# igashov/DiffLinker

Hardware: AMD Instinct MI355X
Metric: molecules/sec (500-step sample_chain) (higher is better)
Workload: dtype f32 (f16x3 split MFMA, fp32 accumulate)

## Files before the change

### difflinker_amd/csrc/egnn_fc.hip

```cpp
#include <hip/hip_runtime.h>
#include <stdint.h>
#include <stdlib.h>
#include <string.h>
#include <math.h>
#include <cmath>

#include <algorithm>
#include <atomic>
#include <vector>

#include "../../include/difflinker_hip.h"
#include "pack_layout.h"


namespace {

constexpr int LDH = 132;
constexpr int NMAX = 55;
constexpr int NQMAX = 2 * NMAX;
constexpr int THREADS = 512;
constexpr int NWAVES = THREADS / 64;
constexpr int GWAVES = 8;
constexpr int GTHREADS = 64 * GWAVES;
constexpr int L_A = 0;
// ... 1242 lines not shown
        for (int t = 0; t < 4; ++t) { acc[t][0] += __uint_as_float(al[t].x ^ ah[t].y); acc[t][1] += __uint_as_float(al[t].z ^ ah[t].w); }
#else
#pragma unroll
        for (int t = 0; t < 4; ++t) acc[t] = mfma16(al[t], b.hi[sl], acc[t]);
#pragma unroll
        for (int t = 0; t < 4; ++t) acc[t] = mfma16(ah[t], b.lo[sl], acc[t]);
#pragma unroll
        for (int t = 0; t < 4; ++t) acc[t] = mfma16(ah[t], b.hi[sl], acc[t]);
#endif
    }
}
template <int SLOT>
__device__ __forceinline__ void st_issue(float* lds0, const float* __restrict__ src, int hw, int lane) {
    typedef const __attribute__((address_space(1))) void* gptr_t;
    typedef __attribute__((address_space(3))) void* lptr_t;
    const float4* s4 = reinterpret_cast<const float4*>(src) + lane;
#ifdef DL_KO_DMA
    (void)s4; (void)lds0; (void)hw;
#else
#pragma unroll
    for (int it = 0; it < ST_PIECES; ++it) {
        const int piece = it * 4 + hw;
        __builtin_amdgcn_global_load_lds((gptr_t)(s4 + piece * 64), (lptr_t)(lds0 + st_slot_off(SLOT) + piece * 256), 16, 0, 0);
    }
#endif
}
template <int HALF>
__device__ __forceinline__ void st_issue_image(const Lds& v, const NextPass& nx, int hw, int lane) {
    typedef const __attribute__((address_space(1))) void* gptr_t;
    typedef __attribute__((address_space(3))) void* lptr_t;
    const float* wimg = nx.base + (nx.equiv ? E_W6T : G_W2T);
    const float* vecs = nx.base + (nx.equiv ? E_VEC : G_VEC) + HID;
    const float* vec4 = nx.base + (nx.equiv ? E_VEC + 4 * HID : G_VEC + 6 * HID);
    if (HALF == 1 && hw < 2) {
        const int t2 = 64 * hw + lane;
        const float4* src = (t2 < 96) ? reinterpret_cast<const float4*>(vecs) + t2 : reinterpret_cast<const float4*>(vec4) + (t2 - 96);
        __builtin_amdgcn_global_load_lds((gptr_t)src, (lptr_t)(v.vec + 256 * hw), 16, 0, 0);
    }
    const float4* s4 = reinterpret_cast<const float4*>(wimg) + lane;
#pragma unroll
    for (int it = 0; it < ST_PIECES; ++it) {
        const int piece = HALF * 32 + it * 4 + hw;
        __builtin_amdgcn_global_load_lds((gptr_t)(s4 + piece * 64), (lptr_t)(v.W + piece * 256), 16, 0, 0);
    }
}
template <int N>
__device__ __forceinline__ void st_wait_vm() {
    if constexpr (N <= 0) asm volatile("s_waitcnt vmcnt(0)" ::: "memory");
    else asm volatile("s_waitcnt vmcnt(%0)" :: "n"(N) : "memory");
}
template <int V>
struct IC { static constexpr int value = V; };

template <bool TEAM, bool POST, bool NEXT_EQ>
__device__ __forceinline__ void stream_phase(const Lds& v, Prof& pf, const AggRegs* ar) {
    constexpr int NC = (POST ? 6 : 0) + 4;
    constexpr int C_P = POST ? 6 : 0;
    const PassCtx cx = pass_ctx(v);
    const LaneIds q = lane_ids(v);
    const int tid = q.tid, w = q.w, lane = q.lane;
    const int nb = cx.nb;
    const int nown = TEAM ? ctx_i(v, TM_NOWN) : nb;
    float* hs = cx.hs;
    const int pass_open = cx.pass + 1;
    const float* wp = ctx_p<const float>(v, CX_WP);
    const int sub = ctx_i(v, CX_SUB);
    const float* g = POST ? cx.g : nullptr;
    const float* nxb = pass_weights(wp, pass_open, sub);
    const NextPass nx = {nxb, NEXT_EQ};
    const float* sc = POST ? g + G_SCALE : nullptr;
    const float* scn = nxb + (NEXT_EQ ? E_SCALE : G_SCALE);
    const float* vecn = nxb + (NEXT_EQ ? E_VEC : G_VEC);
    float* lds0 = v.A - L_A;
    const bool loader = w >= ST_AWAVES;
    const int hw = w - ST_AWAVES, wa = w;
    const int n = lane & 15, kg = lane >> 4;
    const int ta = wa;
    const int l = 16 * ta + n;
    const bool awave = !loader && 16 * ta < nown;
    const bool valid = awave && l < nown;
    const int lc = max(min(l, nown - 1), 0);
    auto chunk_src = [&](int c) -> const float* {
        if (POST && c < C_P) return g + G_ST_POST + c * ST_CHUNK;
        return nxb + (NEXT_EQ ? E_ST_PRE : G_ST_PRE) + (c - C_P) * ST_CHUNK;
    };
    float4 hold[8];
    if (awave) {
#pragma unroll
        for (int ot = 0; ot < 8; ++ot) hold[ot] = *st_tile(hs + HS_HT, ta, ot, lane);
    }
    const int par = cx.par;
    float hmax = 0.f, aggmax = 0.f, s_agg = 1.f, s_t = 1.f, s_hn = 1.f, inv2 = 1.f;
    if constexpr (POST) {
        hmax = __uint_as_float(v.fmax[FM_H0 + par]);
        aggmax = __uint_as_float(v.fmax[FM_AGG]);
        s_agg = scale_for(aggmax);
        const float y3b = cload(sc, SC_L1_W3A) * hmax + cload(sc, SC_L1_W3B) * aggmax + cload(sc, SC_B3);
        s_t = scale_for(y3b);
        const float hnb = hmax + cload(sc, SC_L1_W4) * y3b + cload(sc, SC_B4);
        s_hn = scale_for(hnb);
        if (tid == 0 && (beyond_f16_range(aggmax) || beyond_f16_range(y3b) || beyond_f16_range(hnb))) atomicOr(&v.misc[1], NAN_RANGE | 3);
        inv2 = inv_pow2(s_t * cload(sc, 4));
    }
    const float s_h0 = scale_for(__uint_as_float(v.fmax[FM_H0 + par]));
    const float s_hf = POST ? s_hn : s_h0;
    constexpr int AGG_OFF = st_slot_off(st_slot(3, NC));
    if constexpr (POST) {
#pragma unroll
        for (int k = 0; k < 4; ++k) {
            const int e = tid + THREADS * k;
            if (e < nown * 32) *reinterpret_cast<float4*>(lds0 + AGG_OFF + (e >> 5) * LDH + 4 * (e & 31)) = ar->v[k];
        }
    }
    if (loader) {
        st_issue<st_slot(0, NC)>(lds0, chunk_src(0), hw, lane);
        prof_event(pf, w, lane, 200);
        auto lstep = [&](auto C_) {
            constexpr int C = decltype(C_)::value;
            constexpr int behind = (C >= 1 && C + 1 < NC ? ST_PIECES : 0) + (C == NC - 2 ? ST_PIECES : 0) + (C == NC - 1 ? 2 * ST_PIECES : 0);
            st_wait_vm<behind>();
            fine_event(pf, w, lane, 220 + C);
            lds_barrier();
            fine_event(pf, w, lane, 210 + C);
            if constexpr (C == 0) {
                st_issue<st_slot(1, NC)>(lds0, chunk_src(1), hw, lane);
                st_issue<st_slot(2, NC)>(lds0, chunk_src(2), hw, lane);
            }
            if constexpr (C == 1) st_wait_vm<ST_PIECES>();
            if constexpr (C >= 1 && C + 2 < NC) st_issue<st_slot(C + 2, NC)>(lds0, chunk_src(C + 2), hw, lane);
            if constexpr (C == NC - 3) st_issue_image<0>(v, nx, hw, lane);
            if constexpr (C == NC - 2) st_issue_image<1>(v, nx, hw, lane);
        };
        lstep(IC<0>{}); lstep(IC<1>{}); lstep(IC<2>{}); lstep(IC<3>{});
        if constexpr (NC > 4) { lstep(IC<4>{}); lstep(IC<5>{}); }
        if constexpr (NC > 6) { lstep(IC<6>{}); lstep(IC<7>{}); }
        if constexpr (NC > 8) { lstep(IC<8>{}); lstep(IC<9>{}); }
        fine_event(pf, w, lane, 240);
        lds_barrier();
        prof_event(pf, w, lane, 250);
    } else {
    BOp bh, bagg, bout, bin;
    floatx4 acc[4];
    float4 t0p[4];
    float4 res2[8], bb4[8];
    float4 Pout[8], Qout[8];
    float hm = 0.f;
    float S1 = 1.f;
    if (!TEAM) {
        const float x2 = __uint_as_float(v.fmax[FM_X2]), x02 = __uint_as_float(v.fmax[FM_X02]);
        S1 = fminf(scale_for(4.0f * x2) * scale_for(cload(scn, 6)), scale_for(4.0f * x02) * scale_for(cload(scn, 7)));
    }
    const float live = valid ? 1.0f : 0.0f;
    if (awave) {
        const float sb = s_h0 * live;
#pragma unroll
        for (int sl = 0; sl < 4; ++sl) {
            const float4 a = hold[2 * sl], c4 = hold[2 * sl + 1];
            const float u[8] = {a.x * sb, a.y * sb, a.z * sb, a.w * sb, c4.x * sb, c4.y * sb, c4.z * sb, c4.w * sb};
            split8t(u, bh.hi[sl], bh.lo[sl]);
        }
    }
    prof_event(pf, w, lane, 200);
    auto step = [&](auto C_) {
        constexpr int C = decltype(C_)::value;
        fine_event(pf, w, lane, 230 + C);
        lds_barrier();
        fine_event(pf, w, lane, 210 + C);
        if (!awave) return;
// ... 171 lines not shown
    const int S = TEAM ? ctx_i(v, TM_S) : 1, rank = TEAM ? ctx_i(v, TM_RANK) : 0;
    const bool more = cx.nx.base != nullptr;
    const LaneIds q = lane_ids(v);
    const int tid = q.tid, lane = q.lane;
    lds_barrier();
    const float xscale = (cx.flags & 4) ? 1.0f / float(N) : ((cx.flags & 2) ? ctx_f(v, CX_INVNORM) : 1.0f);
    pair_reduce_equiv<true>(v, nown, nb, tid, xscale);
    if (tid == 0) v.fmax[TEAM ? FM_XOWN : FM_X2] = 0u;
    lds_barrier();
    const float* aggx = v.A - L_A + L_AGGX3;
    float n2 = 0.0f;
    if (tid < nown) {
        const float lm = v.lm[tid];
        const int a = rank + tid * S;
        const bool moves = v.rpos[tid] >= 0;
#pragma unroll
        for (int k = 0; k < 3; ++k) {
            float xn = v.xs[4 * a + k];
            if (moves) {
                xn += aggx[4 * tid + k] * lm;
                v.xs[4 * a + k] = xn;
            }
            n2 = fmaf(xn, xn, n2);
        }
    }
    block_max(&v.fmax[TEAM ? FM_XOWN : FM_X2], n2, lane);
    prof_event(pf, q.w, lane, 34);
    lds_barrier();
    prof_event(pf, q.w, lane, 10);
    if (more) stream_phase<TEAM, false, false>(v, pf, nullptr);
}

template <bool TEAM>
__device__ __forceinline__ void head_phase(const Lds& v, bool v3);

template <int PREC, bool TEAM, bool ATT>
__device__ __forceinline__ void forward_molecule2(const Lds& v, Prof& pf) {
    const int tid = lane_ids(v).tid;
    const int nb = ctx_i(v, 0);
    const int nown = TEAM ? ctx_i(v, TM_NOWN) : nb;
    const int S = TEAM ? ctx_i(v, TM_S) : 1, rank = TEAM ? ctx_i(v, TM_RANK) : 0;
    const float* wp = ctx_p<const float>(v, CX_WP);
    float* hs = ctx_p<float>(v, CX_HS);
    const float tfeat = ctx_f(v, CX_TFEAT);
    const int nf = ctx_i(v, CX_NF), fin = ctx_i(v, CX_FIN);
    const int npass = ctx_i(v, CX_NPASS);
    const int w = __builtin_amdgcn_readfirstlane(tid >> 6);
    const int lane = tid & 63;
    const bool v3 = (PREC != 0) && !TEAM && nown > 32;
    if (tid == 0) { v.misc[CX_PASS] = v3 ? -1 : 0; v.misc[CX_PAR] = 0; v.misc[CX_V3] = v3 ? 1 : 0; }
    if (tid < 8) reinterpret_cast<int*>(v.A - L_A + L_PROG)[tid] = 0;
    if (!TEAM && tid < HID) (v.A - L_A + L_ZROW)[tid] = 0.0f;
    prof_event(pf, w, lane, 1);
    {
        if (tid < 8) v.fmax[tid] = 0u;
        __syncthreads();
    }
    const NextPass first = {wp + OFF_BLOCKS, false};
    if (!v3) stage_next(v, first, w, tid);
    if (tid < 4 * nown) {
        const int l = tid >> 2, k = tid & 3, a = rank + l * S;
        const float xv = (k < 3) ? v.z[l * DMAX + k] : 0.0f;
        v.xs[4 * a + k] = xv;
        v.x0[4 * a + k] = xv;
    }
    {
        float n2 = 0.0f;
        if (tid < nown) {
            const float x0 = v.z[tid * DMAX], x1 = v.z[tid * DMAX + 1], x2 = v.z[tid * DMAX + 2];
            n2 = x0 * x0 + x1 * x1 + x2 * x2;
        }
        const unsigned b = wave_max_u32(__float_as_uint(n2));
        if (lane == 0) {
            if (TEAM) lds_max_u32(&v.fmax[FM_XOWN], b);
            else { lds_max_u32(&v.fmax[FM_X2], b); lds_max_u32(&v.fmax[FM_X02], b); }
        }
    }
    {
        const int f = tid & (HID - 1);
        float wrow[FINP];
        const float4* wsrc = reinterpret_cast<const float4*>(wp + OFF_EMB_W + f * FINP);
#pragma unroll
        for (int q = 0; q < FINP / 4; ++q) {
            const float4 t4 = wsrc[q];
            wrow[4 * q] = t4.x; wrow[4 * q + 1] = t4.y; wrow[4 * q + 2] = t4.z; wrow[4 * q + 3] = t4.w;
        }
        const float be = wp[OFF_EMB_B + f];
        const float* ctxp = ctx_p<const float>(v, CX_CTXP);
        const int ct = ctx_i(v, CX_CT);
        const int nctx = fin - nf - ct;
        float hmax = 0.0f;
        for (int l = tid >> 7; l < nown; l += THREADS / HID) {
            const int pos = v.idx[rank + l * S];
            float acc = be;
#pragma unroll
            for (int k = 0; k < FINP; ++k) {
                float hin = 0.0f;
                if (k < nf) hin = v.z[l * DMAX + 3 + k];
                else if (k < nf + ct) hin = tfeat;
                else if (k < fin) hin = ctxp[pos * nctx + (k - nf - ct)];
                acc = fmaf(wrow[k], hin, acc);
            }
            if (v3) {
                hs[HS_HT + ((((l >> 4) * 8 + (f >> 4)) * 64 + 16 * ((f >> 2) & 3) + (l & 15)) * 4) + (f & 3)] = acc;
            } else {
            v.B[l * LDH + f] = acc;
            {
                const int r = l & 31;
                hs[HS_HT + ((((l >> 5) * 4 + (f >> 5)) * 4 + (r >> 3)) * 64 + (f & 31) + 32 * ((r >> 2) & 1)) * 4 + (r & 3)] = acc;
            }
            }
            hmax = fmaxf(hmax, fabsf(acc));
        }
        block_max(&v.fmax[FM_H0], hmax, lane);
    }
    __syncthreads();
    if (v3) {
        if constexpr (PREC != 0 && !TEAM) {
        if (tid == 0 && beyond_f16_range(__uint_as_float(v.fmax[FM_H0]))) atomicOr(&v.misc[1], NAN_RANGE | 3);
        prof_event(pf, w, lane, 2);
        stream_phase<TEAM, false, false>(v, pf, nullptr);
        const int sub = ctx_i(v, CX_SUB);
#pragma nounroll
        for (int p = 0; p < npass; p += sub + 1) {
#pragma nounroll
            for (int gi = 0; gi < sub; ++gi) gcl_pass3<PREC, TEAM, ATT>(v, pf);
            equiv_pass3<PREC, TEAM>(v, pf);
        }
        prof_event(pf, w, lane, 3);
        __syncthreads();
        head_phase<TEAM>(v, true);
        }
    } else {
    {
        const float s0 = (PREC != 0) ? scale_for(__uint_as_float(v.fmax[FM_H0])) : 1.0f;
        for (int e = tid; e < nown * 32; e += THREADS)
            put_quad<PREC>(v.C + (e >> 5) * LDH, 4 * (e & 31), *reinterpret_cast<const float4*>(v.B + (e >> 5) * LDH + 4 * (e & 31)), s0);
        if (PREC != 0 && tid == 0) {
            v.fmax[FS_HS] = __float_as_uint(s0);
            if (beyond_f16_range(__uint_as_float(v.fmax[FM_H0]))) atomicOr(&v.misc[1], NAN_RANGE | 3);
        }
    }
    __syncthreads();
    prof_event(pf, w, lane, 2);
    {
        PreW2 pw;
        load_pre2(pw, first, w, lane, nown);
        open_pass<PREC, TEAM>(v, nb, nown, first, hs, pf, pw, 0, 0);
    }
    const int sub = ctx_i(v, CX_SUB);
#pragma nounroll
    for (int p = 0; p < npass; p += sub + 1) {
#pragma nounroll
        for (int gi = 0; gi < sub; ++gi) gcl_pass2<PREC, TEAM, ATT>(v, pf);
        equiv_pass2<PREC, TEAM>(v, pf);
    }
    prof_event(pf, w, lane, 3);
    __syncthreads();
    head_phase<TEAM>(v, false);
    }
    prof_event(pf, w, lane, 4);
}

template <bool TEAM>
__device__ __forceinline__ void head_phase(const Lds& v, bool v3) {
    const int tid = lane_ids(v).tid;
    const int nb = ctx_i(v, 0), nf = ctx_i(v, CX_NF);
    const int nown = TEAM ? ctx_i(v, TM_NOWN) : nb;
    const int S = TEAM ? ctx_i(v, TM_S) : 1, rank = TEAM ? ctx_i(v, TM_RANK) : 0;
    const float* wp = ctx_p<const float>(v, CX_WP);
    const float* hs = ctx_p<const float>(v, CX_HS);
    float* eps = v.A;
    int nanbits = 0;
    for (int e = tid; e < nown * nf; e += THREADS) {
        const int a = e / nf, o = e - a * nf;
        const int r = a & 31;
        const float* wo = wp + OFF_OUT_W + o * HID;
        float acc = wp[OFF_OUT_B + o];
        if (v3) {
            const float* hp = hs + HS_HT + ((a >> 4) * 8 * 64 + (a & 15)) * 4;
#pragma unroll
            for (int ot = 0; ot < 8; ++ot)
#pragma unroll
                for (int kg = 0; kg < 4; ++kg) {
                    const float4 hv = *reinterpret_cast<const float4*>(hp + (ot * 64 + 16 * kg) * 4);
                    const float4 wv = *reinterpret_cast<const float4*>(wo + 16 * ot + 4 * kg);
                    acc = fmaf(hv.x, wv.x, acc); acc = fmaf(hv.y, wv.y, acc);
                    acc = fmaf(hv.z, wv.z, acc); acc = fmaf(hv.w, wv.w, acc);
                }
        } else {
        const float* hp = hs + HS_HO + ((a >> 5) * 4 * 16 + (r & 3) + 4 * (r >> 3)) * 64 + 32 * ((r >> 2) & 1);
#pragma unroll
        for (int nt4 = 0; nt4 < 4; ++nt4)
#pragma unroll 8
            for (int q = 0; q < 8; ++q) {
                const float4 hv = *reinterpret_cast<const float4*>(hp + nt4 * 16 * 64 + 4 * q);
                const float4 wv = *reinterpret_cast<const float4*>(wo + 32 * nt4 + 4 * q);
                acc = fmaf(hv.x, wv.x, acc); acc = fmaf(hv.y, wv.y, acc);
                acc = fmaf(hv.z, wv.z, acc); acc = fmaf(hv.w, wv.w, acc);
            }
        }
        (void)r;
        eps[a * DMAX + 3 + o] = acc;
        if (acc != acc) nanbits |= 2;
    }
    if (tid < 4 * nown && (tid & 3) < 3) {
        const int l = tid >> 2, a = rank + l * S;
        const float vel = v.xs[4 * a + (tid & 3)] - v.x0[4 * a + (tid & 3)];
        eps[l * DMAX + (tid & 3)] = vel;
        if (vel != vel) nanbits |= 1;
    }
    if (TEAM && tid == 0 && v.misc[TM_FAIL] != 0) nanbits |= 8;
    if (nanbits) atomicOr(&v.misc[1], nanbits);
// ... 110 lines not shown
        }
        if (tid == 0) {
            if (TEAM) team_init(v, nb, S, rank, p.team_rows + size_t(b) * TEAM_MOL_BYTES, p.team_flags + size_t(b) * TEAM_MAX, p.team_fault);
            ctx_store(v, p.md, N, p.edge_mask ? p.edge_mask + size_t(b) * N * N : nullptr, p.hsave + size_t(blockIdx.x) * HS_STRIDE,
                      p.wpack, p.context ? p.context + size_t(b) * N * p.md.ctx : nullptr, p.t[size_t(b) * p.t_stride], b);
        }
        __syncthreads();
        const int nown = TEAM ? v.misc[TM_NOWN] : nb;
        const float* xh_b = p.xh + size_t(b) * N * D;
        for (int e = tid; e < nown * D; e += THREADS) {
            const int l = e / D, d = e - l * D;
            v.z[l * DMAX + d] = xh_b[v.idx[rank + l * S] * D + d];
        }
        if (tid < nown) v.lm[tid] = p.linker_mask ? p.linker_mask[size_t(b) * N + v.idx[rank + tid * S]] : 1.0f;
        __syncthreads();
        build_receivers(v, nown, tid);
        __syncthreads();
    }
    Prof pf;
    pf.buf = (blockIdx.x == 0) ? p.prof : nullptr;
    pf.n = 0;
    forward_molecule2<PREC, TEAM, ATT>(v, pf);
    {
        const auto* P = kargs<FwdArgs>();
        const int tid = lane_ids(v).tid;
        const int mol = ctx_i(v, CX_MOL), nb = ctx_i(v, 0), N = P->N, D = 3 + P->md.nf;
        const int nown = TEAM ? ctx_i(v, TM_NOWN) : nb;
        const int S2 = TEAM ? ctx_i(v, TM_S) : 1, rank2 = TEAM ? ctx_i(v, TM_RANK) : 0;
        float* out_b = P->out + size_t(mol) * N * D;
        for (int e = tid; e < nown * D; e += THREADS) {
            const int l = e / D, d = e - l * D;
            out_b[v.idx[rank2 + l * S2] * D + d] = v.A[l * DMAX + d];
        }
        if (tid == 0) {
            if (TEAM) { if (v.misc[1]) atomicOr(&P->nan_flags[mol], v.misc[1]); }
            else P->nan_flags[mol] = v.misc[1];
        }
    }
}

struct ChainArgs {
    const float* wpack;
    ModelDims md;
    dl_chain_args a;
    unsigned long long* prof;
    char* team_rows;
    unsigned* team_flags;
    int team_fault;
    float* hsave;
};

template <int PREC, bool TEAM, bool ATT>
__device__ __forceinline__ bool chain_step2(const Lds& v, int q) {
    {
        const auto* P = kargs<ChainArgs>();
        const int tid = lane_ids(v).tid;
        if (tid == 0) {
            const float t = (q == P->a.T) ? 0.0f : P->a.coefs[q].t;
            v.misc[CX_TFEAT] = __float_as_int(t);
        }
        __syncthreads();
    }
    Prof pf;
    pf.buf = (blockIdx.x == 0 && q == 0) ? kargs<ChainArgs>()->prof : nullptr;
    pf.n = 0;
    forward_molecule2<PREC, TEAM, ATT>(v, pf);
    const auto* P = kargs<ChainArgs>();
    const int tid = lane_ids(v).tid;
    const int b = ctx_i(v, CX_MOL), nb = ctx_i(v, 0);
    const int nown = TEAM ? ctx_i(v, TM_NOWN) : nb;
    const int S = TEAM ? ctx_i(v, TM_S) : 1, rank = TEAM ? ctx_i(v, TM_RANK) : 0;
    const int N = P->a.N, nf = P->md.nf, D = 3 + nf, T = P->a.T, K = P->a.keep_frames, B = P->a.B;
    if (v.misc[1] != 0) {
        if (!TEAM) {
            if (tid == 0) { P->a.nan_flags[b] = v.misc[1]; P->a.nan_step[b] = q; }
            return false;
        }
        if (tid == 0) {
            atomicOr(&P->a.nan_flags[b], v.misc[1]);
            atomicCAS(&P->a.nan_step[b], -1, q);
        }
    }
    const bool decode = (q == T);
    dl_step_coef cf;
    if (decode) { cf.t = 0.0f; cf.alpha_ts = 1.0f; cf.c_eps = 0.0f; cf.sigma = 0.0f; }
    else cf = P->a.coefs[q];
    const float* noise_x = P->a.noise_x;
    const float* noise_h = P->a.noise_h;
    const float* fragm = P->a.fragment_mask;
    const bool philox = (noise_x == nullptr);
    const unsigned gmol = unsigned(P->a.mol_offset + (P->a.mol_index ? P->a.mol_index[b] : b));
    const unsigned long long seed = P->a.noise_seed;
    const size_t frame = size_t(B) * N * D;
    const size_t nx_stride = size_t(B) * N * 3, nh_stride = size_t(B) * N * nf;
    float* chain_b = P->a.chain + size_t(b) * N * D;
    const float norm_x = P->a.norm_x, norm_h = P->a.norm_h, bias_h = P->a.bias_h;
    const float inv_alpha0 = P->a.inv_alpha0, sigma0 = P->a.sigma0, sigma_x = P->a.sigma_x;
    const int s = T - 1 - q;
    const int widx = decode ? 0 : (s * K) / T;
    const bool last_writer = (s == 0) || (((s - 1) * K) / T != widx);
    const bool write = !decode && last_writer && widx != 0;
    for (int e = tid; e < nown * D; e += THREADS) {
        const int l = e / D, d = e - l * D;
        const int pos = v.idx[rank + l * S];
        const size_t n = size_t(b) * N + pos;
        const float lm = v.lm[l], fr = v.frag[l];
        const float zt = v.z[l * DMAX + d];
        const float eh = __fmul_rn(v.A[l * DMAX + d], lm);
        float nz;
        if (philox) nz = philox_normal(seed, gmol, unsigned(pos), unsigned(q + 1), unsigned(d));
        else nz = (d < 3) ? noise_x[(q + 1) * nx_stride + n * 3 + d] : noise_h[(q + 1) * nh_stride + n * nf + d - 3];
        float zn;
        if (!decode) {
            const float mu = __fsub_rn(__fdiv_rn(zt, cf.alpha_ts), __fmul_rn(cf.c_eps, eh));
            const float zs = __fadd_rn(mu, __fmul_rn(cf.sigma, __fmul_rn(nz, lm)));
            zn = __fadd_rn(__fmul_rn(zt, fr), __fmul_rn(zs, lm));
            if (write) {
                const float o = (d < 3) ? __fmul_rn(zn, norm_x) : __fadd_rn(__fmul_rn(zn, norm_h), bias_h);
                chain_b[widx * frame + pos * D + d] = o;
            }
        } else {
            const float mu = __fmul_rn(inv_alpha0, __fsub_rn(zt, __fmul_rn(sigma0, eh)));
            const float xh = __fadd_rn(mu, __fmul_rn(sigma_x, __fmul_rn(nz, lm)));
            const float zz = __fadd_rn(__fmul_rn(zt, fr), __fmul_rn(xh, lm));
            zn = (d < 3) ? __fmul_rn(zz, norm_x) : __fadd_rn(__fmul_rn(zz, norm_h), bias_h);
        }
        v.z[l * DMAX + d] = zn;
    }
    (void)fragm;
    if (TEAM && tid == 0) v.misc[1] = 0;
    __syncthreads();
    return true;
}

template <bool TEAM>
__device__ __forceinline__ bool chain_begin(const ChainArgs& p, const Lds& v, int b, int rank, int S, int qb, char* rows,
                                            unsigned* flags) {
    const dl_chain_args& g = p.a;
    const int tid = threadIdx.x;
    const int N = g.N, nf = p.md.nf, D = 3 + nf, K = g.keep_frames, B = g.B;
    const int limit = TEAM ? NQMAX : NMAX;
    if (g.skip_flags && g.skip_flags[b] != 0) return false;
    const int8_t* nm = g.node_mask + size_t(b) * N;
    const size_t frame = size_t(B) * N * D;
    float* chain_b = g.chain + size_t(b) * N * D;
    const int nb = compact_atoms(v, nm, N, tid);
    if (rank == 0) {
        if (tid == 0) {
            if (TEAM) { if (nb > limit) atomicOr(&g.nan_flags[b], 4); }
            else { g.nan_flags[b] = (nb > limit) ? 4 : 0; g.nan_step[b] = -1; }
        }
        for (int kf = 0; kf < K; ++kf)
            for (int e = tid; e < N * D; e += THREADS)
                if (nm[e / D] == 0 || nb > limit) chain_b[kf * frame + e] = 0.0f;
    }
    if (nb > limit || nb == 0) return false;
    if (tid == 0) {
        if (TEAM) team_init(v, nb, S, rank, rows, flags, p.team_fault);
        ctx_store(v, p.md, N, g.edge_mask ? g.edge_mask + size_t(b) * N * N : nullptr, p.hsave + size_t(blockIdx.x) * HS_STRIDE,
                  p.wpack, g.context ? g.context + size_t(b) * N * p.md.ctx : nullptr, 0.0f, b);
    }
    __syncthreads();
    const int nown = TEAM ? v.misc[TM_NOWN] : nb;
    if (tid < nown) {
        const size_t n = size_t(b) * N + v.idx[rank + tid * S];
        v.lm[tid] = g.linker_mask[n];
        v.frag[tid] = g.fragment_mask[n];
    }
    __syncthreads();
    build_receivers(v, nown, tid);
    const bool philox = (g.noise_x == nullptr);
    const unsigned gmol = unsigned(g.mol_offset + (g.mol_index ? g.mol_index[b] : b));
    for (int e = tid; e < nown * D; e += THREADS) {
        const int l = e / D, d = e - l * D;
        const int pos = v.idx[rank + l * S];
        const size_t n = size_t(b) * N + pos;
        float val, eps0;
        if (d < 3) { val = __fdiv_rn(g.x[n * 3 + d], g.norm_x); eps0 = philox ? 0.0f : g.noise_x[n * 3 + d]; }
        else { val = __fdiv_rn(__fsub_rn(g.h[n * nf + d - 3], g.bias_h), g.norm_h); eps0 = philox ? 0.0f : g.noise_h[n * nf + d - 3]; }
        if (philox) eps0 = philox_normal(g.noise_seed, gmol, unsigned(pos), 0u, unsigned(d));
        const float lm = v.lm[l];
        float z0 = __fadd_rn(__fmul_rn(val, v.frag[l]), __fmul_rn(__fmul_rn(eps0, lm), lm));
        if (qb > 0) z0 = g.z_state[n * D + d];
        v.z[l * DMAX + d] = z0;
    }
    __syncthreads();
    return true;
}

template <bool TEAM>
__device__ __forceinline__ void chain_end(const Lds& v, int qe, int T) {
    if (qe <= T) {
        const auto* P = kargs<ChainArgs>();
        const int tid = lane_ids(v).tid;
        const int b = ctx_i(v, CX_MOL), nb = ctx_i(v, 0), D = 3 + P->md.nf, N = P->a.N;
        const int nown = TEAM ? ctx_i(v, TM_NOWN) : nb;
        const int S = TEAM ? ctx_i(v, TM_S) : 1, rank = TEAM ? ctx_i(v, TM_RANK) : 0;
        for (int e = tid; e < nown * D; e += THREADS) {
            const int l = e / D, d = e - l * D;
            P->a.z_state[(size_t(b) * N + v.idx[rank + l * S]) * D + d] = v.z[l * DMAX + d];
        }
        return;
    }
    {
        const auto* P = kargs<ChainArgs>();
        const int tid = lane_ids(v).tid;
        const int b = ctx_i(v, CX_MOL), nb = ctx_i(v, 0), nf = P->md.nf, D = 3 + nf;
        const int nown = TEAM ? ctx_i(v, TM_NOWN) : nb;
        const int S = TEAM ? ctx_i(v, TM_S) : 1, rank = TEAM ? ctx_i(v, TM_RANK) : 0;
        if (tid < nown) {
            const int l = tid;
            float* o = P->a.chain + size_t(b) * P->a.N * D + v.idx[rank + l * S] * D;
            o[0] = v.z[l * DMAX + 0]; o[1] = v.z[l * DMAX + 1]; o[2] = v.z[l * DMAX + 2];
// ... 976 lines not shown
```

### difflinker_amd/edm.py

```python
import ctypes
import functools
import os
import threading
import warnings

import numpy as np
import torch
import torch.nn.functional as F

from . import _lib, utils
from .egnn import Dynamics, DynamicsWithPockets
from .noise import PredefinedNoiseSchedule


SPLIT_CHAIN_DEFAULT = os.environ.get('DIFFLINKER_SPLIT_CHAIN', '1') == '1'


def compute_units(dev):
    return torch.cuda.get_device_properties(dev).multi_processor_count


@functools.lru_cache(maxsize=None)
def xcd_layout(bs):
    ln = -(-bs // 16)
# ... 76 lines not shown
        helpers = rest[:len(owners)]
        q_end = [n_calls] * len(sizes)
        for o, hp in zip(owners, helpers):
            arrive = n_calls * c1[hp] * (1.0 + margin)
            q_end[o] = int(min(max(-(-arrive // c1[o]), 1), n_calls - 1))
        plan = (q_end, owners, helpers)
    with _CACHE_LOCK:
        if len(_PLAN_CACHE) > 64:
            _PLAN_CACHE.clear()
        _PLAN_CACHE[key] = plan
    return plan


def join_makespan(plan, sizes, linkers, n_calls, n_layers, sublayers):
    q_end, owners, helpers = plan
    c1 = [forward_cost(n, l, n_layers, sublayers, 1) for n, l in zip(sizes, linkers)]
    end = [n_calls * c for c in c1]
    for o, hp in zip(owners, helpers):
        start = max(q_end[o] * c1[o], end[hp])
        end[o] = start + (n_calls - q_end[o]) * forward_cost(sizes[o], linkers[o], n_layers, sublayers, 2)
    return max(end)


class EDM(torch.nn.Module):
    def __init__(
            self,
            dynamics,
            in_node_nf: int,
            n_dims: int,
            timesteps: int = 1000,
            noise_schedule='learned',
            noise_precision=1e-4,
            loss_type='vlb',
            norm_values=(1., 1., 1.),
            norm_biases=(None, 0., 0.),
    ):
        super().__init__()
        if noise_schedule == 'learned':
            raise NotImplementedError("noise_schedule='learned' (GammaNetwork) is training-only and out of scope; "
                                      'released configs use polynomial_2')
        self.gamma = PredefinedNoiseSchedule(noise_schedule, timesteps=timesteps, precision=noise_precision)
        self.dynamics = dynamics
        self.in_node_nf = in_node_nf
        self.n_dims = n_dims
        self.T = timesteps
        self.norm_values = norm_values
        self.norm_biases = norm_biases
        self.noise_source = 'torch'
        self.noise_seed = 0
        self.coef_batch = None
        self.team_batch = None
        self.overflow_teams = True
        self.split_chain = SPLIT_CHAIN_DEFAULT
        self.last_route = None

    @staticmethod
    def _side_stream(dev):
        key = dev.index if dev.index is not None else torch.cuda.current_device()
        with _CACHE_LOCK:
            if key not in _SIDE_STREAMS:
                _SIDE_STREAMS[key] = torch.cuda.Stream(device=dev)
            return _SIDE_STREAMS[key]

    @staticmethod
    def _side_workspace(key, need, dev):
        with _CACHE_LOCK:
            ws = _SIDE_WORKSPACE.get(key)
            if ws is None or ws.numel() < need:
                ws = _SIDE_WORKSPACE[key] = torch.empty(need, dtype=torch.uint8, device=dev)
            return ws

    def forward(self, x, h, node_mask, fragment_mask, linker_mask, edge_mask, context=None, *, t_int=None, noise=None,
                mol_offset=0):
        self._check_no_grad()
        rows, t_int_d = self._loss_rows(x, h, node_mask, fragment_mask, linker_mask, edge_mask, context, t_int, noise,
                                        mol_offset)
        return self._reduce_loss_rows(rows, t_int_d)

    _inpainting = False

    def _check_no_grad(self):
        if torch.is_grad_enabled() and any(p.requires_grad for p in self.dynamics.parameters()):
            raise NotImplementedError('EDM.forward evaluates the loss without a backward pass (training is out of scope): '
                                      'wrap the call in torch.no_grad()')

    def _loss_rows(self, x, h, node_mask, fragment_mask, linker_mask, edge_mask, context, t_int, noise, mol_offset,
                   train_state=None):
        dev = x.device
        if dev.type != 'cuda':
            raise _lib.HipLibraryError(f'{type(self).__name__}.forward runs on the HIP device only (no CPU fallback): '
                                       f'got tensors on {dev}')
        lib = _lib.load()
        bs, n = x.size(0), x.size(1)
        nf, T = self.in_node_nf, int(self.T)
        f32 = lambda t_, shape: t_.reshape(shape).to(dev, torch.float32).contiguous()
        xn, hn = self.normalize(x, h)
        xh = torch.cat([xn, hn], dim=2).to(torch.float32).contiguous()
        nm = f32(node_mask, (bs, n))
        fm = f32(fragment_mask, (bs, n)) if fragment_mask is not None else None
        lm = f32(linker_mask, (bs, n)) if linker_mask is not None else None
        philox = self.noise_source == 'philox'
        if mol_offset and not philox and (t_int is None or noise is None):
            raise NotImplementedError("a shard of a batch (mol_offset) needs noise_source='philox' or explicit t_int and noise: "
                                      'the torch.randn stream is a property of the whole batch')
        if t_int is None and not philox:
            t_int = torch.randint(0, T + 1, size=(bs, 1), device=dev)
# ... 359 lines not shown
                raise err
        finally:
            self.coef_batch = pinned
            self.team_batch = pinned_team
        return chain

    def _sample_chain_fused(self, x, h, node_mask, fragment_mask, linker_mask, edge_mask, context, keep_frames, noise_bank,
                            seed, mol_offset, mol_index, team=None):
        dev = x.device
        lib = _lib.load()
        bs, n = x.size(0), x.size(1)
        nf, T = self.in_node_nf, self.T
        handle = self.dynamics.hip_model(dev)
        philox = noise_bank is None
        noise_x, noise_h = (None, None) if philox else noise_bank
        coefs, (inv_alpha0, sigma0, sigma_x) = self.step_coefficients(bs)
        coefs = coefs.to(dev)
        f32 = lambda t_, shape: t_.reshape(shape).to(torch.float32).contiguous()
        xs, hs = f32(x, (bs, n, self.n_dims)), f32(h, (bs, n, nf))
        nm = node_mask.reshape(bs, n).to(torch.int8).contiguous()
        fm, lm = f32(fragment_mask, (bs, n)), f32(linker_mask, (bs, n))
        em = edge_mask.reshape(bs, n, n).to(torch.int8).contiguous() if edge_mask is not None else None
        ctx = f32(context, (bs, n, self.dynamics.context_node_nf)) if context is not None else None
        n_real = nm.ne(0).sum(1)
        order = torch.argsort(n_real, descending=True, stable=True).to(torch.int32).contiguous()
        cus = compute_units(dev)
        if 16 <= bs <= cus:
            order = order[xcd_layout(bs).to(dev)].contiguous()
        chain = torch.zeros((keep_frames, bs, n, self.n_dims + nf), device=dev)
        flags = torch.zeros(bs, dtype=torch.int32, device=dev)
        steps = torch.full((bs,), -1, dtype=torch.int32, device=dev)
        if team is None:
            team = 1 if self.dynamics._no_teams else \
                self.dynamics.team_for(bs if self.team_batch is None else max(bs, int(self.team_batch)), dev)
        over = 0
        if team == 1 and self.overflow_teams and self.team_batch is None and not self.dynamics._no_teams:
            if cus < bs <= cus + cus // 4:
                over = bs - cus
                team2 = 4 if over <= cus // 16 else 2
                while team2 > 1 and int(lib.dl_team_max(over)) < team2:
                    team2 //= 2
                if team2 < 2:
                    over = 0
            elif cus < bs < 2 * cus and not getattr(EDM, '_warned_off_sweet_spot', False):
                EDM._warned_off_sweet_spot = True
                warnings.warn(f'EDM.sample_chain: a batch of {bs} molecules on {cus} compute units runs one molecule per compute unit '
                              f'for the whole chain, so the {bs - cus} molecules beyond {cus} start only when others have finished; '
                              f'batches of k x {cus} molecules (or up to {cus + cus // 4}, whose surplus is sampled by teams beside '
                              f'the rest) use the chip evenly', RuntimeWarning, stacklevel=3)
        ws, ws_bytes = self.dynamics.workspace(bs - over, team, dev)

        plan = join = None
        if team == 1 and over == 0 and self.split_chain and self.team_batch is None and not self.dynamics._no_teams \
                and bs <= cus and T >= 20:
            counts = torch.stack([n_real, lm.ne(0).sum(1)]).cpu()
            sizes_h, linkers_h = counts[0].tolist(), counts[1].tolist()
            if max(sizes_h) <= int(lib.dl_max_atoms()) and min(sizes_h) > 0:
                sub = int(getattr(self.dynamics, 'inv_sublayers', 2))
                plan = split_plan(sizes_h, linkers_h, T + 1, cus, self.dynamics.n_layers, sub)
                if plan is not None and int(lib.dl_team_max(len(plan[1]))) < 2:
                    plan = None
                if plan is not None:
                    join = join_plan(sizes_h, linkers_h, T + 1, cus, self.dynamics.n_layers, sub)
                    if join is not None:
                        plan = None
        self.last_route = 'join' if join is not None else 'two_launch' if plan is not None else 'overflow_teams' if over else 'one'
        q_end_t = z_state = None
        if plan is not None or join is not None:
            q_end_t = torch.tensor((join or plan)[0], dtype=torch.int32, device=dev)
            z_state = torch.empty((bs, n, self.n_dims + nf), device=dev)

        def chain_args(flags_, steps_, team_, ws_, ws_bytes_, order_, first, count, q_begin=None, q_end=None, skip=None):
            return _lib.DLChainArgs(
                q_begin=q_begin.data_ptr() if q_begin is not None else None, q_end=q_end.data_ptr() if q_end is not None else None,
                z_state=z_state.data_ptr() if z_state is not None else None, skip_flags=skip.data_ptr() if skip is not None else None,
                B=bs, N=n, T=T, keep_frames=keep_frames,
                x=xs.data_ptr(), h=hs.data_ptr(), node_mask=nm.data_ptr(), fragment_mask=fm.data_ptr(),
                linker_mask=lm.data_ptr(), edge_mask=em.data_ptr() if em is not None else None,
                context=ctx.data_ptr() if ctx is not None else None,
                noise_x=None if philox else noise_x.data_ptr(), noise_h=None if philox else noise_h.data_ptr(),
                noise_seed=seed, mol_offset=int(mol_offset), team=team_, coefs=coefs.data_ptr(),
                inv_alpha0=inv_alpha0, sigma0=sigma0, sigma_x=sigma_x,
                norm_x=float(self.norm_values[0]), norm_h=float(self.norm_values[1]), bias_h=float(self.norm_biases[1]),
                chain=chain.data_ptr(), nan_flags=flags_.data_ptr(), nan_step=steps_.data_ptr(), order=order_.data_ptr(),
                workspace=ws_.data_ptr(), workspace_bytes=ws_bytes_,
                mol_index=mol_index.data_ptr() if mol_index is not None else None, order_first=first, order_count=count)

        def side_launch(after, team_, order_, first, count, q_begin=None):
            side = self._side_stream(dev)
            flags2 = torch.empty(bs, dtype=torch.int32, device=dev)
            steps2 = torch.empty(bs, dtype=torch.int32, device=dev)
            need = int(lib.dl_workspace_bytes(count, team_))
            ws2 = self._side_workspace((dev.index, 'teams'), need, dev)
            skip = flags if q_begin is not None else None
            args2 = chain_args(flags2, steps2, team_, ws2, need, order_, first, count, q_begin=q_begin, skip=skip)
            side.wait_event(after)
            _lib.check(lib.dl_sample_chain_fc(handle, ctypes.byref(args2), ctypes.c_void_p(side.cuda_stream)),
                       'dl_sample_chain_fc (teams, beside the main launch)')
            done = torch.cuda.Event()
            done.record(side)
            cur.wait_event(done)
            for t_ in (xs, hs, nm, fm, lm, em, ctx, coefs, order_, chain, noise_x, noise_h, mol_index, q_begin, z_state, skip):
                if t_ is not None:
                    t_.record_stream(side)
            return flags | flags2, torch.where(steps2 >= 0, steps2, steps)

        args = chain_args(flags, steps, team, ws, ws_bytes, order, 0, bs - over if over else 0, q_end=q_end_t)
# ... 327 lines not shown
```

Measured before the change: 581.8.

## Overlap first-pass weight streaming with embedding in v3 forward entry

For the v3 path (large molecules), loader waves now start streaming the first pass's weights into LDS and enter stream_phase in a loader-only role. Meanwhile the compute waves build the input features, compute the embedding, and hand their tile registers straight into stream_phase in a compute-only role, so the old full-block syncs and the stage_next step are skipped. The time feature is now written at the end of the previous chain step, and the launch context is seeded with the first step's t, which removes one barrier per step. The added barrier pairing between the two roles is delicate and could deadlock or race if it gets out of sync.

```diff
diff --git a/difflinker_amd/csrc/egnn_fc.hip b/difflinker_amd/csrc/egnn_fc.hip
--- a/difflinker_amd/csrc/egnn_fc.hip
+++ b/difflinker_amd/csrc/egnn_fc.hip
@@ -1318,8 +1318,8 @@
 template <int V>
 struct IC { static constexpr int value = V; };
 
-template <bool TEAM, bool POST, bool NEXT_EQ>
-__device__ __forceinline__ void stream_phase(const Lds& v, Prof& pf, const AggRegs* ar) {
+template <bool TEAM, bool POST, bool NEXT_EQ, int ROLE = 0>
+__device__ __forceinline__ void stream_phase(const Lds& v, Prof& pf, const AggRegs* ar, const float4* hold_in = nullptr) {
     constexpr int NC = (POST ? 6 : 0) + 4;
     constexpr int C_P = POST ? 6 : 0;
     const PassCtx cx = pass_ctx(v);
@@ -1338,7 +1338,7 @@
     const float* scn = nxb + (NEXT_EQ ? E_SCALE : G_SCALE);
     const float* vecn = nxb + (NEXT_EQ ? E_VEC : G_VEC);
     float* lds0 = v.A - L_A;
-    const bool loader = w >= ST_AWAVES;
+    const bool loader = ROLE == 1 ? true : ROLE == 2 ? false : w >= ST_AWAVES;
     const int hw = w - ST_AWAVES, wa = w;
     const int n = lane & 15, kg = lane >> 4;
     const int ta = wa;
@@ -1353,7 +1353,7 @@
     float4 hold[8];
     if (awave) {
 #pragma unroll
-        for (int ot = 0; ot < 8; ++ot) hold[ot] = *st_tile(hs + HS_HT, ta, ot, lane);
+        for (int ot = 0; ot < 8; ++ot) hold[ot] = (ROLE == 2) ? hold_in[ot] : *st_tile(hs + HS_HT, ta, ot, lane);
     }
     const int par = cx.par;
     float hmax = 0.f, aggmax = 0.f, s_agg = 1.f, s_t = 1.f, s_hn = 1.f, inv2 = 1.f;
@@ -1379,7 +1379,7 @@
         }
     }
     if (loader) {
-        st_issue<st_slot(0, NC)>(lds0, chunk_src(0), hw, lane);
+        if constexpr (ROLE != 1) st_issue<st_slot(0, NC)>(lds0, chunk_src(0), hw, lane);
         prof_event(pf, w, lane, 200);
         auto lstep = [&](auto C_) {
             constexpr int C = decltype(C_)::value;
@@ -1657,12 +1657,106 @@
     if (tid < 8) reinterpret_cast<int*>(v.A - L_A + L_PROG)[tid] = 0;
     if (!TEAM && tid < HID) (v.A - L_A + L_ZROW)[tid] = 0.0f;
     prof_event(pf, w, lane, 1);
+    if (v3) {
+        if constexpr (PREC != 0 && !TEAM) {
+        const int sub = ctx_i(v, CX_SUB);
+        if (w >= ST_AWAVES) {
+            st_issue<st_slot(0, 4)>(v.A - L_A, pass_weights(wp, 0, sub) + G_ST_PRE, w - ST_AWAVES, lane);
+            lds_barrier();
+            lds_barrier();
+            prof_event(pf, w, lane, 2);
+            stream_phase<TEAM, false, false, 1>(v, pf, nullptr);
+        } else {
+            constexpr int ATH = ST_AWAVES * 64;
+            static_assert(FINP == 16 && 4 * NMAX <= ATH && HID <= ATH, "forward entry: thread maps");
+            if (tid < 8) v.fmax[tid] = 0u;
+            const int f = tid & (HID - 1);
+            float wrow[FINP];
+            const float4* wsrc = reinterpret_cast<const float4*>(wp + OFF_EMB_W + f * FINP);
+#pragma unroll
+            for (int q = 0; q < FINP / 4; ++q) {
+                const float4 t4 = wsrc[q];
+                wrow[4 * q] = t4.x; wrow[4 * q + 1] = t4.y; wrow[4 * q + 2] = t4.z; wrow[4 * q + 3] = t4.w;
+            }
+            const float be = wp[OFF_EMB_B + f];
+            float* hin_rows = v.C;
+            {
+                const float* ctxp = ctx_p<const float>(v, CX_CTXP);
+                const int ct = ctx_i(v, CX_CT);
+                const int nctx = fin - nf - ct;
+                for (int e = tid; e < nown * FINP; e += ATH) {
+                    const int l = e >> 4, k = e & 15;
+                    float hin = 0.0f;
+                    if (k < nf) hin = v.z[l * DMAX + 3 + k];
+                    else if (k < nf + ct) hin = tfeat;
+                    else if (k < fin) hin = ctxp[v.idx[l] * nctx + (k - nf - ct)];
+                    hin_rows[e] = hin;
+                }
+            }
+            lds_barrier();
+            if (tid < 4 * nown) {
+                const int l = tid >> 2, k = tid & 3;
+                const float xv = (k < 3) ? v.z[l * DMAX + k] : 0.0f;
+                v.xs[4 * l + k] = xv;
+                v.x0[4 * l + k] = xv;
+            }
+            {
+                float n2 = 0.0f;
+                if (tid < nown) {
+                    const float x0 = v.z[tid * DMAX], x1 = v.z[tid * DMAX + 1], x2 = v.z[tid * DMAX + 2];
+                    n2 = x0 * x0 + x1 * x1 + x2 * x2;
+                }
+                const unsigned b = wave_max_u32(__float_as_uint(n2));
+                if (lane == 0) { lds_max_u32(&v.fmax[FM_X2], b); lds_max_u32(&v.fmax[FM_X02], b); }
+            }
+            {
+                float hmax = 0.0f;
+                for (int l = tid >> 7; l < nown; l += ATH / HID) {
+                    const float4* hr = reinterpret_cast<const float4*>(hin_rows + l * FINP);
+                    float acc = be;
+#pragma unroll
+                    for (int q = 0; q < FINP / 4; ++q) {
+                        const float4 h4 = hr[q];
+                        acc = fmaf(wrow[4 * q], h4.x, acc); acc = fmaf(wrow[4 * q + 1], h4.y, acc);
+                        acc = fmaf(wrow[4 * q + 2], h4.z, acc); acc = fmaf(wrow[4 * q + 3], h4.w, acc);
+                    }
+                    v.B[l * LDH + f] = acc;
+                    hmax = fmaxf(hmax, fabsf(acc));
+                }
+                block_max(&v.fmax[FM_H0], hmax, lane);
+            }
+            lds_barrier();
+            if (tid == 0 && beyond_f16_range(__uint_as_float(v.fmax[FM_H0]))) atomicOr(&v.misc[1], NAN_RANGE | 3);
+            float4 hold[8];
+            if (16 * w < nown) {
+                const int lc = min(16 * w + (lane & 15), nown - 1), kg = lane >> 4;
+#pragma unroll
+                for (int ot = 0; ot < 8; ++ot) {
+                    hold[ot] = *reinterpret_cast<const float4*>(v.B + lc * LDH + 16 * ot + 4 * kg);
+                    *st_tile(hs + HS_HT, w, ot, lane) = hold[ot];
+                }
+            }
+            prof_event(pf, w, lane, 2);
+            stream_phase<TEAM, false, false, 2>(v, pf, nullptr, hold);
+        }
+#pragma nounroll
+        for (int p = 0; p < npass; p += sub + 1) {
+#pragma nounroll
+            for (int gi = 0; gi < sub; ++gi) gcl_pass3<PREC, TEAM, ATT>(v, pf);
+            equiv_pass3<PREC, TEAM>(v, pf);
+        }
+        prof_event(pf, w, lane, 3);
+        head_phase<TEAM>(v, true);
+        }
+        prof_event(pf, w, lane, 4);
+        return;
+    }
     {
         if (tid < 8) v.fmax[tid] = 0u;
         __syncthreads();
     }
     const NextPass first = {wp + OFF_BLOCKS, false};
-    if (!v3) stage_next(v, first, w, tid);
+    stage_next(v, first, w, tid);
     if (tid < 4 * nown) {
         const int l = tid >> 2, k = tid & 3, a = rank + l * S;
         const float xv = (k < 3) ? v.z[l * DMAX + k] : 0.0f;
@@ -1706,37 +1800,16 @@
                 else if (k < fin) hin = ctxp[pos * nctx + (k - nf - ct)];
                 acc = fmaf(wrow[k], hin, acc);
             }
-            if (v3) {
-                hs[HS_HT + ((((l >> 4) * 8 + (f >> 4)) * 64 + 16 * ((f >> 2) & 3) + (l & 15)) * 4) + (f & 3)] = acc;
-            } else {
             v.B[l * LDH + f] = acc;
             {
                 const int r = l & 31;
                 hs[HS_HT + ((((l >> 5) * 4 + (f >> 5)) * 4 + (r >> 3)) * 64 + (f & 31) + 32 * ((r >> 2) & 1)) * 4 + (r & 3)] = acc;
             }
-            }
             hmax = fmaxf(hmax, fabsf(acc));
         }
         block_max(&v.fmax[FM_H0], hmax, lane);
     }
     __syncthreads();
-    if (v3) {
-        if constexpr (PREC != 0 && !TEAM) {
-        if (tid == 0 && beyond_f16_range(__uint_as_float(v.fmax[FM_H0]))) atomicOr(&v.misc[1], NAN_RANGE | 3);
-        prof_event(pf, w, lane, 2);
-        stream_phase<TEAM, false, false>(v, pf, nullptr);
-        const int sub = ctx_i(v, CX_SUB);
-#pragma nounroll
-        for (int p = 0; p < npass; p += sub + 1) {
-#pragma nounroll
-            for (int gi = 0; gi < sub; ++gi) gcl_pass3<PREC, TEAM, ATT>(v, pf);
-            equiv_pass3<PREC, TEAM>(v, pf);
-        }
-        prof_event(pf, w, lane, 3);
-        __syncthreads();
-        head_phase<TEAM>(v, true);
-        }
-    } else {
     {
         const float s0 = (PREC != 0) ? scale_for(__uint_as_float(v.fmax[FM_H0])) : 1.0f;
         for (int e = tid; e < nown * 32; e += THREADS)
@@ -1763,7 +1836,6 @@
     prof_event(pf, w, lane, 3);
     __syncthreads();
     head_phase<TEAM>(v, false);
-    }
     prof_event(pf, w, lane, 4);
 }
 
@@ -1980,15 +2052,6 @@
 
 template <int PREC, bool TEAM, bool ATT>
 __device__ __forceinline__ bool chain_step2(const Lds& v, int q) {
-    {
-        const auto* P = kargs<ChainArgs>();
-        const int tid = lane_ids(v).tid;
-        if (tid == 0) {
-            const float t = (q == P->a.T) ? 0.0f : P->a.coefs[q].t;
-            v.misc[CX_TFEAT] = __float_as_int(t);
-        }
-        __syncthreads();
-    }
     Prof pf;
     pf.buf = (blockIdx.x == 0 && q == 0) ? kargs<ChainArgs>()->prof : nullptr;
     pf.n = 0;
@@ -2013,6 +2076,7 @@
     dl_step_coef cf;
     if (decode) { cf.t = 0.0f; cf.alpha_ts = 1.0f; cf.c_eps = 0.0f; cf.sigma = 0.0f; }
     else cf = P->a.coefs[q];
+    const float tnext = (q + 1 < T) ? P->a.coefs[q + 1].t : 0.0f;
     const float* noise_x = P->a.noise_x;
     const float* noise_h = P->a.noise_h;
     const float* fragm = P->a.fragment_mask;
@@ -2056,7 +2120,10 @@
         v.z[l * DMAX + d] = zn;
     }
     (void)fragm;
-    if (TEAM && tid == 0) v.misc[1] = 0;
+    if (tid == 0) {
+        if (TEAM) v.misc[1] = 0;
+        v.misc[CX_TFEAT] = __float_as_int(tnext);
+    }
     __syncthreads();
     return true;
 }
@@ -2086,7 +2153,8 @@
     if (tid == 0) {
         if (TEAM) team_init(v, nb, S, rank, rows, flags, p.team_fault);
         ctx_store(v, p.md, N, g.edge_mask ? g.edge_mask + size_t(b) * N * N : nullptr, p.hsave + size_t(blockIdx.x) * HS_STRIDE,
-                  p.wpack, g.context ? g.context + size_t(b) * N * p.md.ctx : nullptr, 0.0f, b);
+                  p.wpack, g.context ? g.context + size_t(b) * N * p.md.ctx : nullptr,
+                  qb < g.T ? g.coefs[qb].t : 0.0f, b);
     }
     __syncthreads();
     const int nown = TEAM ? v.misc[TM_NOWN] : nb;
diff --git a/difflinker_amd/edm.py b/difflinker_amd/edm.py
--- a/difflinker_amd/edm.py
+++ b/difflinker_amd/edm.py
@@ -152,6 +152,7 @@
         self.team_batch = None
         self.overflow_teams = True
         self.split_chain = SPLIT_CHAIN_DEFAULT
+        self.split_chain_min_T = 20
         self.last_route = None
 
     @staticmethod
@@ -617,7 +618,7 @@
 
         plan = join = None
         if team == 1 and over == 0 and self.split_chain and self.team_batch is None and not self.dynamics._no_teams \
-                and bs <= cus and T >= 20:
+                and bs <= cus and T >= self.split_chain_min_T:
             counts = torch.stack([n_real, lm.ne(0).sum(1)]).cpu()
             sizes_h, linkers_h = counts[0].tolist(), counts[1].tolist()
             if max(sizes_h) <= int(lib.dl_max_atoms()) and min(sizes_h) > 0:
```

Result: no change. 583.4, median of 6 (+0.3%).
